# ffs97/deep-mixture-vae

Hardware: AMD Instinct MI355X
Metric: images/sec (train), MNIST K=10 z=64 batch=4096/GPU bf16 (higher is better)
Workload: dtype bf16; 1 GPU; configs[1]: DMVAE MLP 784-500-500-(2000|2000)-z64/K10-2000-500-500-784, one ELBO training step (gather+fwd+loss+bwd+Adam), synthetic rows resident in HBM; per_gpu_batch=4096, global_batch=4096, parallelism=dp1, rccl_ranks=0, multi_rank_rccl_verified_before_this_run=False, hip_graph=True, float_atomics=False, update=adam fused into the dW launch, mode=exact (expectation over q(c|x), priors.py:130-145)

## Files before the change

### deep-mixture-vae_amd/csrc/gemm_bf16.hip

```cpp
#include <algorithm>
#include <cmath>
#include <functional>
#include <map>
#include <mutex>
#include <string>
#include <vector>

#include "gemm_tile.h"
#include "measure.h"

MEAS_TABLES_BF16

namespace dmvae {

template <int BM, int BN, int LAYOUT, int EPI, int NSTAGE, int NW, int BKT = BK, bool CONV = false, bool BONLY = false>
__device__ __forceinline__ void gemm_bf16_body(const GemmArgs& a, const int bid_raw, const int gstart, const int nwg, bf16_t* smem,
                                               const dmvae_adam_ctx* ac = nullptr, const int kslice = -1) {
    constexpr bool A_KC = (LAYOUT != DMVAE_GEMM_DW);
    constexpr bool B_KC = (LAYOUT == DMVAE_GEMM_DX);
    constexpr int A_ELEMS = BM * BKT, B_ELEMS = BN * BKT, STAGE = A_ELEMS + B_ELEMS;
    constexpr int WM = NW / 2;
    constexpr int TM = BM / (16 * WM), TN = BN / 32;
    static_assert(!BONLY || (LAYOUT == DMVAE_GEMM_DW && EPI == DMVAE_EPI_STORE_F32 && !CONV), "bias-only strips: dense DW / STORE_F32");
    constexpr int LOADS = ((BONLY ? 0 : BM) + BN) * BKT / (512 * NW);
    static_assert(NSTAGE >= 2 && NSTAGE <= 8 && LOADS * (NSTAGE - 1) <= 63, "ring depth / vmcnt range");

    MEAS_ANAT(0);
    const int tid = threadIdx.x, lane = tid & 63;
    const int wave = __builtin_amdgcn_readfirstlane(tid >> 6);
    const int wm = wave >> 1, wn = wave & 1;
    const int tiles_n = a.N / BN;
    const int bid = nwg < 0 ? bid_raw : xcd_run_index(gstart + bid_raw, gstart, gstart + nwg);
    int tm, tn;
    {
        const int tiles_m = a.M / BM, gm_max = a.group_m;
        const int gsz = gm_max * tiles_n, grp = bid / gsz, first = grp * gm_max;
        const int gm = min(tiles_m - first, gm_max), in = bid - grp * gsz;
        tm = first + in % gm;
        tn = in / gm;
    }
    const int m0 = tm * BM, n0 = tn * BN;
    const int kbeg = (kslice >= 0 ? kslice : (int)blockIdx.y) * a.k_split;
    const int nk = a.k_split / BKT;

    const bf16_t* Ag = reinterpret_cast<const bf16_t*>(a.A);
    const bf16_t* Bg = reinterpret_cast<const bf16_t*>(a.B);
    if (!A_KC && CONV)
        Ag += ((int64_t)kbeg - (a.conv_p + 1)) * a.lda;
    else
        Ag += A_KC ? ((int64_t)m0 * a.lda + kbeg) : ((int64_t)kbeg * a.lda + m0);
    Bg += B_KC ? ((int64_t)n0 * a.ldb + kbeg) : ((int64_t)kbeg * a.ldb + n0);
    const int64_t stepA = A_KC ? (int64_t)BKT : (int64_t)BKT * a.lda;
    const int64_t stepB = B_KC ? (int64_t)BKT : (int64_t)BKT * a.ldb;

    f32x4 acc[TM][TN];
#pragma unroll
    for (int i = 0; i < TM; ++i)
#pragma unroll
        for (int j = 0; j < TN; ++j) acc[i][j] = f32x4{0.f, 0.f, 0.f, 0.f};
    constexpr bool DW = (LAYOUT == DMVAE_GEMM_DW);
    const bool do_bias = DW && !MEAS_NO_BIAS_MFMA && a.epi.out2 != nullptr && (tm == 0 || BONLY);
    f32x4 bacc[TN];
#pragma unroll
    for (int j = 0; j < TN; ++j) bacc[j] = f32x4{0.f, 0.f, 0.f, 0.f};
    const s16x8 ones_bits = {0x3F80, 0x3F80, 0x3F80, 0x3F80, 0x3F80, 0x3F80, 0x3F80, 0x3F80};
    const bf16x8 ones = __builtin_bit_cast(bf16x8, ones_bits);

    unsigned goA[BM * BKT / (512 * NW)], goB[BN * BKT / (512 * NW)];
    stage_offsets<BM, A_KC, NW, BKT>(a.lda, wave, lane, goA);
    stage_offsets<BN, B_KC, NW, BKT>(a.ldb, wave, lane, goB);
    unsigned selA[BM * BKT / (512 * NW)];
#pragma unroll
    for (int i = 0; i < BM * BKT / (512 * NW); ++i) selA[i] = 0;
    if constexpr (CONV) {
        static_assert(A_KC || BM == 64, "conv-mode weight gradient: 64-row tiles");
#pragma unroll
        for (int i = 0; i < BM * BKT / (512 * NW); ++i) {
            const int row = i * (8 * NW) + wave * 8 + (lane >> 3);
            if constexpr (A_KC) {
                const int k = swz_kc(row, lane & 7) * 8;
                selA[i] = (unsigned)(k / a.conv_c);
                goA[i] = 2u * (unsigned)(row * (int)a.lda + k % a.conv_c);
            } else {
                const int m = m0 + swz_nc<64>(row, lane & 7) * 8;
                const int tap = min(m / a.conv_c, 8);
                goA[i] = 2u * (unsigned)((row + (tap / 3 - 1) * a.conv_p + (tap % 3 - 1) + a.conv_p + 1) * (int)a.lda + m % a.conv_c);
            }
        }
    }
    unsigned short foA[BKT / 32][TM][2], foB[BKT / 32][TN][2];
#pragma unroll
    for (int ks = 0; ks < BKT / 32; ++ks) {
#pragma unroll
        for (int i = 0; i < TM; ++i) frag_offsets<BM, A_KC>(wm * (BM / WM) + i * 16, ks, lane, foA[ks][i][0], foA[ks][i][1]);
#pragma unroll
        for (int j = 0; j < TN; ++j) frag_offsets<BN, B_KC>(wn * (BN / 2) + j * 16, ks, lane, foB[ks][j][0], foB[ks][j][1]);
    }
    const unsigned lds_w = __builtin_amdgcn_readfirstlane(
        (unsigned)(size_t)((__attribute__((address_space(3))) bf16_t*)smem) + 1024u * (unsigned)wave);

    int cv_tap = 0, cv_c0 = 0;
    int64_t cv_off = 0;
    unsigned cv_delta = 0;
    auto issue = [&](int t, int slot) {
        const int tc = t;
        const unsigned s = lds_w + 2u * (unsigned)(slot * STAGE);
        if constexpr (A_KC && CONV) {
            if (t < nk) {
                const int t0 = min(cv_tap, 8), t1 = min(cv_tap + 1, 8);
                cv_off = conv_tap_offset(t0, cv_c0, a.conv_p, a.lda);
                cv_delta = (unsigned)(2 * (int)(conv_tap_offset(t1, 0, a.conv_p, a.lda) - conv_tap_offset(t0, 0, a.conv_p, a.lda)));
                cv_c0 += BKT;
                while (cv_c0 >= a.conv_c) { cv_c0 -= a.conv_c; ++cv_tap; }
            }
            unsigned o[BM * BKT / (512 * NW)];
#pragma unroll
            for (int i = 0; i < BM * BKT / (512 * NW); ++i) o[i] = goA[i] + selA[i] * cv_delta;
            glds_tile(Ag + cv_off, o, s, 1024u * NW);
        } else if constexpr (!BONLY) {
            glds_tile(Ag + tc * stepA, goA, s, 1024u * NW);
        }
        glds_tile(Bg + tc * stepB, goB, s + 2u * A_ELEMS, 1024u * NW);
    };
    auto rd = [&](int slot, int ks, bf16x8 (&af)[TM], bf16x8 (&bfr)[TN]) {
        const bf16_t* As = smem + slot * STAGE;
        const bf16_t* Bs = As + A_ELEMS;
        if constexpr (MEAS_NO_LDS_READ) {
#pragma unroll
            for (int i = 0; i < TM; ++i) af[i] = ones;
#pragma unroll
            for (int j = 0; j < TN; ++j) bfr[j] = ones;
        } else {
            if constexpr (!BONLY) {
#pragma unroll
                for (int i = 0; i < TM; ++i) af[i] = read_frag<A_KC>(As, foA[ks][i][0], foA[ks][i][1]);
            }
#pragma unroll
            for (int j = 0; j < TN; ++j) bfr[j] = read_frag<B_KC>(Bs, foB[ks][j][0], foB[ks][j][1]);
        }
    };
    auto mma = [&](const bf16x8 (&af)[TM], const bf16x8 (&bfr)[TN]) {
        if constexpr (MEAS_NO_MFMA) {
#pragma unroll
            for (int i = 0; i < TM; ++i) asm volatile("" ::"v"(af[i]));
#pragma unroll
            for (int j = 0; j < TN; ++j) asm volatile("" ::"v"(bfr[j]));
        } else if constexpr (!BONLY) {
            __builtin_amdgcn_s_setprio(1);
#pragma unroll
            for (int i = 0; i < TM; ++i)
#pragma unroll
                for (int j = 0; j < TN; ++j)
                    acc[i][j] = __builtin_amdgcn_mfma_f32_16x16x32_bf16(bfr[j], af[i], acc[i][j], 0, 0, 0);
            __builtin_amdgcn_s_setprio(0);
        }
        if constexpr (DW) {
            if (do_bias) {
#pragma unroll
                for (int j = 0; j < TN; ++j) bacc[j] = __builtin_amdgcn_mfma_f32_16x16x32_bf16(bfr[j], ones, bacc[j], 0, 0, 0);
            }
        }
    };

    static_assert(BKT == 64, "the pipelined loop handles two 32-deep sub-steps per ring slot");
    bf16x8 f0a[TM], f0b[TN], f1a[TM], f1b[TN];
    constexpr int NQ = BM * (BN / 4) / (64 * NW);
    float4 target[EPI == DMVAE_EPI_BIAS_RECON ? NQ : 1];
    unsigned target_zero = 0;
    if constexpr (EPI == DMVAE_EPI_BIAS_RECON) {
        const bool tg = (a.epi.recon_kind & 0x100) != 0;
        int64_t tfirst = 0;
        if (tg) {
            const dmvae_state* tst = reinterpret_cast<const dmvae_state*>(a.epi.aux2);
            tfirst = tst ? (int64_t)tst->batch_cursor * a.epi.d_off : a.epi.ld1;
        }
        if (tg) {
            const int32_t* perm = reinterpret_cast<const int32_t*>(a.epi.aux1);
            int64_t src[NQ];
            bool ok[NQ];
#pragma unroll
            for (int q = 0; q < NQ; ++q) {
                const int idx = q * (64 * NW) + tid;
                const int m = m0 + idx / (BN / 4), n = n0 + (idx % (BN / 4)) * 4;
                const int64_t sr = tfirst + m;
                ok[q] = m < a.epi.m_valid && n + 3 < (int)a.epi.ld0 && sr >= 0 && sr < a.epi.ld2;
                src[q] = ok[q] ? sr : 0;
            }
            if (perm) {
#pragma unroll
                for (int q = 0; q < NQ; ++q) src[q] = (int64_t)perm[src[q]];
            }
#pragma unroll
            for (int q = 0; q < NQ; ++q) {
                const int idx = q * (64 * NW) + tid;
                const int n = n0 + (idx % (BN / 4)) * 4;
                ok[q] = ok[q] && src[q] >= 0 && src[q] < a.epi.ld2;
                target[q] = *reinterpret_cast<const float4*>(reinterpret_cast<const float*>(a.epi.aux0) + (ok[q] ? src[q] * a.epi.ld0 + n : 0));
                if (!ok[q]) target_zero |= 1u << q;
            }
        } else {
#pragma unroll
            for (int q = 0; q < NQ; ++q) {
                const int idx = q * (64 * NW) + tid;
                const int ml = idx / (BN / 4), c = idx % (BN / 4);
                target[q] = *reinterpret_cast<const float4*>(reinterpret_cast<const float*>(a.epi.aux0) + (int64_t)(m0 + ml) * a.epi.ld0 + n0 + c * 4);
            }
        }
    }
    constexpr bool LAT_PRE = EPI == DMVAE_EPI_LATENT && NQ <= 4;
    float lat[LAT_PRE ? NQ : 1][12];
    if constexpr (LAT_PRE) {
#pragma unroll
        for (int q = 0; q < NQ; ++q) {
            const int idx = q * (64 * NW) + tid;
            const int ml = idx / (BN / 4), c = idx % (BN / 4);
            loadf4(a.epi.aux0, (int64_t)(m0 + ml) * a.epi.ld0 + n0 + c * 4, lat[q]);
            loadf4(a.epi.aux1, (int64_t)(m0 + ml) * a.epi.ld1 + n0 + c * 4, lat[q] + 4);
            loadf4(a.epi.aux2, (int64_t)(m0 + ml) * a.epi.ld2 + n0 + c * 4, lat[q] + 8);
        }
    }
    constexpr bool HAS_BIAS = (EPI == DMVAE_EPI_BIAS_RELU || EPI == DMVAE_EPI_BIAS_F32 || EPI == DMVAE_EPI_BIAS_SIGMOID || EPI == DMVAE_EPI_BIAS_RECON);
    static_assert((64 * NW) % (BN / 4) == 0, "a thread keeps its column block across the epilogue's passes");
    float bq[4] = {0.f, 0.f, 0.f, 0.f};
    if constexpr (HAS_BIAS) loadf4(a.epi.bias, n0 + (tid % (BN / 4)) * 4, bq);
    uint2 gate[EPI == DMVAE_EPI_RELU_MASK ? NQ : 1];
    if constexpr (EPI == DMVAE_EPI_RELU_MASK) {
#pragma unroll
        for (int q = 0; q < NQ; ++q) {
            const int idx = q * (64 * NW) + tid;
            const int ml = idx / (BN / 4), c = idx % (BN / 4);
            if constexpr (MEAS_NO_MASK_READ) gate[q] = make_uint2(0x3f803f80u, 0x3f803f80u);
            else gate[q] = *reinterpret_cast<const uint2*>(reinterpret_cast<const bf16_t*>(a.epi.aux0) + (int64_t)(m0 + ml) * a.epi.ld0 + n0 + c * 4);
        }
    }
#pragma unroll
    for (int t = 0; t < NSTAGE; ++t)
        if (t < nk) issue(t, t);
    if (nk >= NSTAGE) wait_vmcnt<LOADS*(NSTAGE - 1)>();
    else wait_vmcnt<0>();
    __builtin_amdgcn_s_barrier();
    MEAS_ANAT(1);
    rd(0, 0, f0a, f0b);
    for (int kt = 0; kt < nk; kt += NSTAGE) {
#pragma unroll
        for (int s = 0; s < NSTAGE; ++s) {
            if (kt + s < nk) {
                rd(s, 1, f1a, f1b);
                mma(f0a, f0b);
                asm volatile("s_waitcnt lgkmcnt(0)" ::: "memory");
                if (kt + s + NSTAGE <= nk) wait_vmcnt<LOADS*(NSTAGE - 2)>();
                else wait_vmcnt<0>();
                __builtin_amdgcn_s_barrier();
                if constexpr (!MEAS_NO_KLOOP_LOADS) {
                    if (kt + s + NSTAGE < nk) issue(kt + s + NSTAGE, s);
                }
                if (kt + s + 1 < nk) rd((s + 1) % NSTAGE, 0, f0a, f0b);
                mma(f1a, f1b);
            }
        }
    }
    wait_vmcnt<0>();
    __builtin_amdgcn_s_barrier();
    MEAS_KLOOP_END();
    MEAS_ANAT(2);

    float loss = 0.f;
    const int li = lane & 15, g = lane >> 4;
    constexpr int CH = BN / 4, NT = 64 * NW;
    static_assert(BM * BN * 4 <= NSTAGE * STAGE * 2, "fp32 tile must fit in the ring");
    dmvae_epilogue epi_s = a.epi;
    if constexpr (EPI == DMVAE_EPI_STORE_F32 && (CONV || LAYOUT == DMVAE_GEMM_DW)) {
        const int ys = kslice >= 0 ? kslice : (int)blockIdx.y;
        epi_s.out = reinterpret_cast<float*>(epi_s.out) + (int64_t)ys * a.slab_stride;
        if (epi_s.out2) epi_s.out2 = reinterpret_cast<float*>(epi_s.out2) + (int64_t)ys * a.slab_stride2;
    }
    float* ct = reinterpret_cast<float*>(smem);
    if constexpr (MEAS_NO_EPILOGUE) {
#pragma unroll
        for (int i = 0; i < TM; ++i)
#pragma unroll
            for (int j = 0; j < TN; ++j) asm volatile("" ::"v"(acc[i][j]));
    } else if constexpr (!BONLY) {
#pragma unroll
    for (int i = 0; i < TM; ++i)
#pragma unroll
        for (int j = 0; j < TN; ++j) {
            const int ml = wm * (BM / WM) + i * 16 + li;
            const int c = (wn * (BN / 2) + j * 16) / 4 + g;
            *reinterpret_cast<f32x4*>(ct + ml * BN + ((c ^ (ml & 7)) << 2)) = acc[i][j];
        }
    __syncthreads();
    constexpr int KSPLIT_MAX_S = 8;
    constexpr bool KSLICE_OK = !CONV && LAYOUT != DMVAE_GEMM_DW && BM * BN <= 4096 && NW <= 4 && BM * BN * 4 + 16 <= NSTAGE * STAGE * 2 &&
                               (EPI == DMVAE_EPI_BIAS_RELU || EPI == DMVAE_EPI_RELU_MASK || EPI == DMVAE_EPI_BIAS_F32 || EPI == DMVAE_EPI_LATENT);
    if constexpr (KSLICE_OK) {
        if (a.tick != nullptr && gridDim.y > 1) {
            const int S = (int)gridDim.y, tile_lin = tm * tiles_n + tn;
            constexpr int Q = BM * BN;
            static_assert(KSPLIT_MAX_S == 8, "the combine issues eight loads per quad");
            f32x4* slab0 = reinterpret_cast<f32x4*>(a.ws) + (int64_t)tile_lin * S * (Q / 4);
            const f32x4* ct4 = reinterpret_cast<const f32x4*>(ct);
            for (int q = tid; q < Q / 4; q += 64 * NW) {
                const f32x4 v = ct4[q];
                f32x4* dst = slab0 + (int64_t)blockIdx.y * (Q / 4) + q;
                asm volatile("global_store_dwordx4 %0, %1, off sc1" ::"v"(dst), "v"(v) : "memory");
            }
            asm volatile("s_waitcnt vmcnt(0)" ::: "memory");
            __syncthreads();
            int* flag = reinterpret_cast<int*>(ct + BM * BN);
            if (tid == 0) *flag = __hip_atomic_fetch_add(a.tick + tile_lin, 1, __ATOMIC_RELAXED, __HIP_MEMORY_SCOPE_AGENT);
            __syncthreads();
            if (*flag != S - 1) return;
            for (int q = tid; q < Q / 4; q += 64 * NW) {
                const f32x4 *p0, *p1, *p2, *p3, *p4, *p5, *p6, *p7;
                auto at = [&](int sl) { return slab0 + (int64_t)(sl < S ? sl : S - 1) * (Q / 4) + q; };
                p0 = at(0); p1 = at(1); p2 = at(2); p3 = at(3); p4 = at(4); p5 = at(5); p6 = at(6); p7 = at(7);
                f32x4 u0, u1, u2, u3, u4, u5, u6, u7;
                asm volatile(
                    "global_load_dwordx4 %0, %8, off sc1\n\tglobal_load_dwordx4 %1, %9, off sc1\n\tglobal_load_dwordx4 %2, %10, off sc1\n\tglobal_load_dwordx4 %3, %11, off sc1\n\t"
                    "global_load_dwordx4 %4, %12, off sc1\n\tglobal_load_dwordx4 %5, %13, off sc1\n\tglobal_load_dwordx4 %6, %14, off sc1\n\tglobal_load_dwordx4 %7, %15, off sc1\n\t"
                    "s_waitcnt vmcnt(0)"
                    : "=&v"(u0), "=&v"(u1), "=&v"(u2), "=&v"(u3), "=&v"(u4), "=&v"(u5), "=&v"(u6), "=&v"(u7)
                    : "v"(p0), "v"(p1), "v"(p2), "v"(p3), "v"(p4), "v"(p5), "v"(p6), "v"(p7)
                    : "memory");
                f32x4 v = u0;
                if (1 < S) v += u1;
                if (2 < S) v += u2;
                if (3 < S) v += u3;
                if (4 < S) v += u4;
                if (5 < S) v += u5;
                if (6 < S) v += u6;
                if (7 < S) v += u7;
                reinterpret_cast<f32x4*>(ct)[q] = v;
            }
            if (tid == 0) __hip_atomic_store(a.tick + tile_lin, 0, __ATOMIC_RELAXED, __HIP_MEMORY_SCOPE_AGENT);
            __syncthreads();
        }
    }
    if constexpr (EPI == DMVAE_EPI_ADAM && !CONV) {
        constexpr int NQE = BM * CH / NT;
        constexpr int NB = NQE % 4 == 0 ? 4 : (NQE % 2 == 0 ? 2 : 1);
        const unsigned base = (unsigned)((reinterpret_cast<const float*>(a.epi.out) - ac->grad) + (int64_t)m0 * a.epi.ldo + n0);
#ifndef DMVAE_ADAM_EPI_BATCHWISE
#ifdef DMVAE_ADAM_EPI_NB
        constexpr int PNB = NQE % DMVAE_ADAM_EPI_NB == 0 ? DMVAE_ADAM_EPI_NB : NB, PDEPTH = DMVAE_ADAM_EPI_DEPTH;
#else
        constexpr int PNB = NB, PDEPTH = 2;
#endif
        adam_pipelined<PNB, NQE / PNB, PDEPTH>(*ac,
            [&](int i, int b) {
                const int idx = (i * PNB + b) * NT + tid;
                return base + (unsigned)(idx / CH) * (unsigned)a.epi.ldo + (unsigned)(idx % CH) * 4u;
            },
            [&](int i, int b, float (&gv)[4]) {
                const int idx = (i * PNB + b) * NT + tid;
                const int ml = idx / CH, c = idx % CH;
                const f32x4 t = *reinterpret_cast<const f32x4*>(ct + ml * BN + ((c ^ (ml & 7)) << 2));
                gv[0] = t[0]; gv[1] = t[1]; gv[2] = t[2]; gv[3] = t[3];
            });
#else
#pragma unroll
        for (int q0 = 0; q0 < NQE; q0 += NB) {
            unsigned off[NB];
#pragma unroll
            for (int b = 0; b < NB; ++b) {
                const int idx = (q0 + b) * NT + tid;
                off[b] = base + (unsigned)(idx / CH) * (unsigned)a.epi.ldo + (unsigned)(idx % CH) * 4u;
            }
            adam_quads<NB>(*ac, off, [&](int b, float (&gv)[4]) {
                const int idx = (q0 + b) * NT + tid;
                const int ml = idx / CH, c = idx % CH;
                const f32x4 t = *reinterpret_cast<const f32x4*>(ct + ml * BN + ((c ^ (ml & 7)) << 2));
                gv[0] = t[0]; gv[1] = t[1]; gv[2] = t[2]; gv[3] = t[3];
            });
        }
#endif
    } else
#pragma unroll
    for (int q = 0; q < BM * CH / NT; ++q) {
        const int idx = q * NT + tid;
        const int ml = idx / CH, c = idx % CH;
        bool padcol = false;
        if constexpr (CONV) {
            padcol = n0 + c * 4 >= a.epi.n_valid;
            if (padcol && !(EPI == DMVAE_EPI_STORE_F32 && a.slab_stride)) continue;
        }
        const f32x4 t = *reinterpret_cast<const f32x4*>(ct + ml * BN + ((c ^ (ml & 7)) << 2));
        float v[4] = {t[0], t[1], t[2], t[3]};
        if (padcol) { v[0] = 0.f; v[1] = 0.f; v[2] = 0.f; v[3] = 0.f; }
        if constexpr (EPI == DMVAE_EPI_ADAM) {
            const int64_t off = (reinterpret_cast<const float*>(a.epi.out) - ac->grad) + (int64_t)(m0 + ml) * a.epi.ldo + n0 + c * 4;
            adam_quad(*ac, off, v);
        } else if constexpr (EPI == DMVAE_EPI_RELU_MASK) {
            const uint2 y = gate[q];
            v[0] = __uint_as_float(y.x << 16) > 0.f ? v[0] : 0.f;
            v[1] = __uint_as_float(y.x & 0xffff0000u) > 0.f ? v[1] : 0.f;
            v[2] = __uint_as_float(y.y << 16) > 0.f ? v[2] : 0.f;
            v[3] = __uint_as_float(y.y & 0xffff0000u) > 0.f ? v[3] : 0.f;
            ActIO<bf16_t>::store4(a.epi.out, (int64_t)(m0 + ml) * a.epi.ldo + n0 + c * 4, v);
        } else if constexpr (EPI == DMVAE_EPI_BIAS_RECON) {
            const bool tz = (target_zero >> q) & 1u;
            const float xq[4] = {tz ? 0.f : target[q].x, tz ? 0.f : target[q].y, tz ? 0.f : target[q].z, tz ? 0.f : target[q].w};
            epilogue_quad<EPI, bf16_t>(a.epi, m0 + ml, n0 + c * 4, v, loss, xq, nullptr, bq);
        } else if constexpr (LAT_PRE) {
            epilogue_quad<EPI, bf16_t>(a.epi, m0 + ml, n0 + c * 4, v, loss, lat[q]);
        } else {
            epilogue_quad<EPI, bf16_t>(epi_s, m0 + ml, n0 + c * 4, v, loss, nullptr, nullptr, HAS_BIAS ? bq : nullptr);
        }
    }
    }
    if constexpr (DW) {
        if (do_bias && wm == 0 && li == 0) {
            float* db = reinterpret_cast<float*>(epi_s.out2);
#pragma unroll
            for (int j = 0; j < TN; ++j) {
                const int n = n0 + wn * (BN / 2) + j * 16 + g * 4;
                if constexpr (CONV) {
                    if (n >= a.epi.n_valid) {
                        if (EPI == DMVAE_EPI_STORE_F32 && a.slab_stride2) *reinterpret_cast<float4*>(db + n) = make_float4(0.f, 0.f, 0.f, 0.f);
                        continue;
                    }
                }
                if constexpr (EPI == DMVAE_EPI_ATOMIC_F32) {
#pragma unroll
                    for (int e = 0; e < 4; ++e) atomicAdd(db + n + e, bacc[j][e]);
                } else if constexpr (EPI == DMVAE_EPI_ADAM) {
                    float v[4] = {bacc[j][0], bacc[j][1], bacc[j][2], bacc[j][3]};
                    adam_quad(*ac, (db - ac->grad) + n, v);
                } else {
                    *reinterpret_cast<float4*>(db + n) = make_float4(bacc[j][0], bacc[j][1], bacc[j][2], bacc[j][3]);
                }
            }
        }
    }
    if constexpr (EPI == DMVAE_EPI_BIAS_RECON) {
        float* red = reinterpret_cast<float*>(smem);
        lds_barrier();
        const float t = block_sum_waves<NW>(loss, red);
        constexpr int CM = BM / 64, CN = BN / 64;
        if (tid < CM * CN) a.epi.partials[(tm * CM + tid / CN) * (a.N / 64) + tn * CN + tid % CN] = tid == 0 ? t : 0.f;
    }
    MEAS_ANAT_DRAIN();
}

template <int BM, int BN, int LAYOUT, int EPI, int NSTAGE, int NW>
__global__ __launch_bounds__(64 * NW, (EPI == DMVAE_EPI_BIAS_RECON ? 1 : NW / 2)) void gemm_bf16_kernel(GemmArgs a) {
    __shared__ __attribute__((aligned(16))) bf16_t smem[NSTAGE * (BM + BN) * BK];
    gemm_bf16_body<BM, BN, LAYOUT, EPI, NSTAGE, NW>(a, blockIdx.x, 0, gridDim.x, smem);
}

template <int BM, int BN, int EPI, int NSTAGE, int NW>
__global__ __launch_bounds__(64 * NW, NW / 2) void gemm_bf16_dx_riders_kernel(GemmArgs a, GemmRiders r) {
    __shared__ __attribute__((aligned(16))) bf16_t smem[NSTAGE * (BM + BN) * BK];
    const int lead = r.nfin + (r.gat_last ? 0 : r.ngat);
    if (blockIdx.y > 0 && ((int)blockIdx.x < lead || (r.gat_last && (int)blockIdx.x >= (int)gridDim.x - r.ngat))) return;
    if (r.gat_last && (int)blockIdx.x >= (int)gridDim.x - r.ngat) {
        if constexpr (MEAS_EMPTY_GATHER_RIDERS) return;
        gather_rows_block<bf16_t, 16>((int)blockIdx.x - ((int)gridDim.x - r.ngat), 64 * NW, r.gat);
        return;
    }
    if ((int)blockIdx.x < r.nfin) {
        if (NW > 4 && threadIdx.x >= 256) return;
        if ((int)blockIdx.x < r.fin.nblocks) step_finalize_block((int)blockIdx.x, r.fin, reinterpret_cast<float(*)[17]>(smem));
        return;
    }
    if ((int)blockIdx.x < lead) {
        if constexpr (MEAS_EMPTY_GATHER_RIDERS) return;
        gather_rows_block<bf16_t, 16>((int)blockIdx.x - r.nfin, 64 * NW, r.gat);
        return;
    }
    gemm_bf16_body<BM, BN, DMVAE_GEMM_DX, EPI, NSTAGE, NW>(a, (int)blockIdx.x - lead, lead, (int)gridDim.x - lead - (r.gat_last ? r.ngat : 0), smem);
}

template <int BM, int BN, int LAYOUT, int EPI, int NSTAGE, int NW>
__global__ __launch_bounds__(64 * NW, NW / 2) void gemm_bf16_conv_kernel(GemmArgs a) {
    __shared__ __attribute__((aligned(16))) bf16_t smem[NSTAGE * (BM + BN) * BK];
    if constexpr (LAYOUT == DMVAE_GEMM_DW) {
        if ((gridDim.y & 7) == 0) {
            const int L = (int)(blockIdx.y * gridDim.x + blockIdx.x), xcd = L & 7, j = L >> 3, T = (int)gridDim.x;
            gemm_bf16_body<BM, BN, LAYOUT, EPI, NSTAGE, NW, BK, true>(a, j % T, 0, -1, smem, nullptr, (j / T) * 8 + xcd);
            return;
        }
    }
    gemm_bf16_body<BM, BN, LAYOUT, EPI, NSTAGE, NW, BK, true>(a, blockIdx.x, 0, gridDim.x, smem);
}

void* gemm_bf16_anatomy() { return MEAS_SYMBOL(g_anat); }
void* gemm_bf16_stamps() { return MEAS_SYMBOL(g_stamps); }
struct GroupedArgs {
    int nprob;
    int kind[DMVAE_MAX_GROUP];
    int start[DMVAE_MAX_GROUP + 1];
    int cls_start[DMVAE_MAX_GROUP], cls_end[DMVAE_MAX_GROUP];
    int nsl[DMVAE_MAX_GROUP];
    GemmArgs p[DMVAE_MAX_GROUP];
    dmvae_adam_ctx adam;
    dmvae_finalize_args fin;
    int lead, lead_work;
    int xcut, xr0[8], xcnt[8];
};
template <int BM, int BN, int LAYOUT, int EPI, int NSTAGE, int NW = 4, bool SHORTK = false>
__global__ __launch_bounds__(64 * NW, NW == 8 ? 4 : 1) void gemm_bf16_grouped_kernel(GroupedArgs g) {
    __shared__ __attribute__((aligned(16))) bf16_t smem[SHORTK ? 2 * (64 + 64) * BK : 3 * (128 + 64) * BK];
    const dmvae_adam_ctx* ac = EPI == DMVAE_EPI_ADAM ? &g.adam : nullptr;
    if constexpr (EPI == DMVAE_EPI_ADAM) {
        if ((int)blockIdx.x < g.lead) {
            if ((int)blockIdx.x >= g.lead_work) return;
            const int64_t n4 = g.adam.seg_n >> 2;
            for (int64_t q = (int64_t)blockIdx.x * (64 * NW) + threadIdx.x; q < n4; q += (int64_t)g.lead_work * (64 * NW)) {
                const int64_t off = g.adam.seg_off + 4 * q;
                const float4 gq = *reinterpret_cast<const float4*>(g.adam.grad + off);
                const float gv[4] = {gq.x, gq.y, gq.z, gq.w};
                adam_quad(g.adam, off, gv);
            }
            return;
        }
    }
    int bx = (int)blockIdx.x;
    if constexpr (EPI == DMVAE_EPI_ADAM) bx -= g.lead;
    if constexpr (EPI == DMVAE_EPI_RELU_MASK) {
        if (bx < g.lead) {
            if (NW > 4 && threadIdx.x >= 256) return;
            if (bx < g.fin.nblocks) step_finalize_block(bx, g.fin, reinterpret_cast<float(*)[17]>(smem));
            return;
        }
        bx -= g.lead;
    }
    int i = 0, item;
    if (g.xcut) {
        const int x = bx & 7, j = bx >> 3;
        if (j >= g.xcnt[x]) return;
        item = g.xr0[x] + j;
    } else {
        while (i + 1 < g.nprob && bx >= g.start[i + 1]) ++i;
        item = g.cls_start[i] + xcd_run_index(bx, g.cls_start[i], g.cls_end[i]);
    }
    i = 0;
    while (i + 1 < g.nprob && item >= g.start[i + 1]) ++i;
    int bid = item - g.start[i];
    const int kind = g.kind[i];
    const int gs = 0, cnt = -1;
    int ksl = -1;
    if (g.nsl[i] > 1) {
        const int tiles_i = (g.start[i + 1] - g.start[i]) / g.nsl[i];
        ksl = bid / tiles_i;
        bid -= ksl * tiles_i;
    }
    MEAS_WG_BEGIN();
    if constexpr (SHORTK) {
        gemm_bf16_body<64, 64, LAYOUT, EPI, 2, NW>(g.p[i], bid, gs, cnt, smem, ac, ksl);
    } else {
        if (kind == 0) gemm_bf16_body<128, 128, LAYOUT, EPI, 2, NW>(g.p[i], bid, gs, cnt, smem, ac, ksl);
        else if (kind == 1) gemm_bf16_body<128, 64, LAYOUT, EPI, 3, NW>(g.p[i], bid, gs, cnt, smem, ac, ksl);
        else if (kind == 3) {
            if constexpr (LAYOUT == DMVAE_GEMM_DW && EPI == DMVAE_EPI_STORE_F32)
                gemm_bf16_body<64, 64, LAYOUT, EPI, 4, NW, BK, false, true>(g.p[i], bid, gs, cnt, smem, ac, ksl);
        }
        else gemm_bf16_body<BM, BN, LAYOUT, EPI, NSTAGE, NW>(g.p[i], bid, gs, cnt, smem, ac, ksl);
    }
    MEAS_WG_END(LAYOUT, kind);
}

static int g_thin = 2;
static int g_group_m = 0;
int gemm_auto_group_m(int tiles_m, int tiles_n, int bm, int bn, double run) {
    if (g_group_m > 0) return g_group_m;
    const double R = run > 0.0 ? run : std::max(1.0, tiles_m * (double)tiles_n / 8.0);
    int gm = (int)(std::sqrt(R * bn / bm) + 0.5);
    const int need = (int)((R + tiles_n - 1) / tiles_n);
    gm = std::max(gm, need);
    return std::max(1, std::min(gm, tiles_m));
}
static int g_shortk = 0;
static int g_conv_short = 2;
static int g_grouped_cls = 1;
static int g_dx_group_nw = 0;
static int g_grouped_mixed = 1;
static int g_grouped_xcut = 0;
template <int BM, int BN, int LAYOUT, int EPI, int NSTAGE, int NW = 4>
static const char* kernel_name(bool grouped) {
    static char nm[2][64];
    static bool init = false;
    if (!init) {
        snprintf(nm[0], 64, "gemm_bf16_kernel<%d, %d, %d, %d, %d, %d>", BM, BN, LAYOUT, EPI, NSTAGE, NW);
        snprintf(nm[1], 64, "gemm_bf16_grouped_kernel<%d, %d, %d, %d, %d, %d>", BM, BN, LAYOUT, EPI, NSTAGE, NW);
        init = true;
    }
    return nm[grouped ? 1 : 0];
}
static double gemm_bytes(const GemmArgs& a, int layout = DMVAE_GEMM_FWD) {
    const int k = a.epi.kind;
    if (k == DMVAE_EPI_ADAM) return 2.0 * ((double)a.M * a.K + (double)a.K * a.N);
    const double osz = (k == DMVAE_EPI_STORE_F32 || k == DMVAE_EPI_ATOMIC_F32 || k == DMVAE_EPI_BIAS_F32 || k == DMVAE_EPI_BIAS_SIGMOID) ? 4.0 : 2.0;
    if (a.conv_c) {
// ... 400 lines not shown
```

### deep-mixture-vae_amd/csrc/gemm_epilogue.h

```cpp
#pragma once
#include "common.h"

namespace dmvae {

struct GemmArgs {
    const void* A; int64_t lda;
    const void* B; int64_t ldb;
    int M, N, K, k_split;
    int group_m;
    int conv_p, conv_c;
    dmvae_epilogue epi;
    float* ws = nullptr; int64_t ws_elems = 0;
    int64_t slab_stride = 0;
    int64_t slab_stride2 = 0;
    float* csum_out = nullptr; int64_t csum_ld = 0;
    const float* csum_in = nullptr; int csum_rows = 0;
    int bias_only = 0;
    int* tick = nullptr;
};

__host__ __device__ __forceinline__ int64_t conv_tap_offset(int tap, int c0, int P, int64_t lda) {
    return (int64_t)((tap / 3 - 1) * P + (tap % 3 - 1)) * lda + c0;
}

template <typename T> struct ActIO;
template <> struct ActIO<bf16_t> {
    static __device__ __forceinline__ void store4(void* base, int64_t off, const float v[4]) {
        uint2 p;
        p.x = pack2bf(v[0], v[1]);
        p.y = pack2bf(v[2], v[3]);
        *reinterpret_cast<uint2*>(reinterpret_cast<bf16_t*>(base) + off) = p;
    }
    static __device__ __forceinline__ void load4(const void* base, int64_t off, float v[4]) {
        const uint2 p = *reinterpret_cast<const uint2*>(reinterpret_cast<const bf16_t*>(base) + off);
        v[0] = __uint_as_float(p.x << 16);
        v[1] = __uint_as_float(p.x & 0xffff0000u);
        v[2] = __uint_as_float(p.y << 16);
        v[3] = __uint_as_float(p.y & 0xffff0000u);
    }
};
template <> struct ActIO<float> {
    static __device__ __forceinline__ void store4(void* base, int64_t off, const float v[4]) {
        *reinterpret_cast<float4*>(reinterpret_cast<float*>(base) + off) = make_float4(v[0], v[1], v[2], v[3]);
    }
    static __device__ __forceinline__ void load4(const void* base, int64_t off, float v[4]) {
        const float4 p = *reinterpret_cast<const float4*>(reinterpret_cast<const float*>(base) + off);
        v[0] = p.x; v[1] = p.y; v[2] = p.z; v[3] = p.w;
    }
};

__device__ __forceinline__ void loadf4(const void* base, int64_t off, float v[4]) {
    ActIO<float>::load4(base, off, v);
}

__device__ __forceinline__ float xent_logits(float l, float x) {
    return fmaxf(l, 0.f) - l * x + log1pf(__expf(-fabsf(l)));
}
__device__ __forceinline__ float sigmoidf_(float l) { return 1.0f / (1.0f + __expf(-l)); }
struct dmvae_gather_args {
    const float* data; int64_t n_rows; int dim; const int32_t* perm;
    int64_t first; int batch, n_valid, B_pad;
    void* out_act; int64_t ld_act; float* out_f32; int64_t ld_f32; int cols_pad;
    const dmvae_state* st;
    int nblocks;
};
template <typename ACT, int U, bool PERM>
__device__ __forceinline__ void gather_rows_pass(const int base, const int nthreads, const int total, const int quads, const int64_t first, const dmvae_gather_args& g) {
    int r[U], c[U];
    int64_t idx[U];
    bool inb[U];
#pragma unroll
    for (int u = 0; u < U; ++u) {
        const int i = base + u * nthreads;
        r[u] = i < total ? i / quads : -1;
        c[u] = i < total ? (i - r[u] * quads) * 4 : 0;
        const int64_t sr = first + r[u];
        inb[u] = r[u] >= 0 && r[u] < g.n_valid && sr >= 0 && sr < g.n_rows;
        idx[u] = inb[u] ? sr : 0;
    }
    if constexpr (PERM) {
#pragma unroll
        for (int u = 0; u < U; ++u) idx[u] = (int64_t)g.perm[idx[u]];
    }
    float4 q[U];
#pragma unroll
    for (int u = 0; u < U; ++u) {
        inb[u] = inb[u] && idx[u] >= 0 && idx[u] < g.n_rows && c[u] < g.dim;
        q[u] = *reinterpret_cast<const float4*>(g.data + (inb[u] ? idx[u] * g.dim + c[u] : 0));
    }
#pragma unroll
    for (int u = 0; u < U; ++u) {
        if (r[u] < 0) continue;
        const float v[4] = {inb[u] ? q[u].x : 0.f, inb[u] ? q[u].y : 0.f, inb[u] ? q[u].z : 0.f, inb[u] ? q[u].w : 0.f};
        if (g.out_act) ActIO<ACT>::store4(g.out_act, (int64_t)r[u] * g.ld_act + c[u], v);
        if (g.out_f32) ActIO<float>::store4(g.out_f32, (int64_t)r[u] * g.ld_f32 + c[u], v);
    }
}
template <typename ACT, int U = 8>
__device__ __forceinline__ void gather_rows_block(const int bx, const int nthreads, const dmvae_gather_args& g) {
    int64_t first = g.first;
    if (g.st) first = (int64_t)g.st->batch_cursor * g.batch;
    const int quads = g.cols_pad >> 2;
    const int total = g.B_pad * quads;
    if (g.dim % 4 == 0 && (reinterpret_cast<uintptr_t>(g.data) & 15) == 0 && g.n_rows > 0) {
        for (int base = bx * nthreads * U + (int)threadIdx.x; base < total; base += g.nblocks * nthreads * U) {
            if (g.perm) gather_rows_pass<ACT, U, true>(base, nthreads, total, quads, first, g);
            else gather_rows_pass<ACT, U, false>(base, nthreads, total, quads, first, g);
        }
        return;
    }
    for (int i = bx * nthreads + (int)threadIdx.x; i < total; i += g.nblocks * nthreads) {
        const int r = i / quads, c = (i - r * quads) * 4;
        float v[4] = {0.f, 0.f, 0.f, 0.f};
        if (r < g.n_valid) {
            int64_t src = first + r;
            if (g.perm) src = (src >= 0 && src < g.n_rows) ? (int64_t)g.perm[src] : -1;
            if (src >= 0 && src < g.n_rows) {
                const float* p = g.data + src * g.dim + c;
#pragma unroll
                for (int j = 0; j < 4; ++j) v[j] = (c + j < g.dim) ? p[j] : 0.f;
            }
        }
        if (g.out_act) ActIO<ACT>::store4(g.out_act, (int64_t)r * g.ld_act + c, v);
        if (g.out_f32) ActIO<float>::store4(g.out_f32, (int64_t)r * g.ld_f32 + c, v);
    }
}

struct GemmRiders {
    dmvae_finalize_args fin; int nfin = 0;
    dmvae_gather_args gat; int ngat = 0;
    int gat_last = 0;
};

__device__ __forceinline__ void xent_sigmoid(float l, float x, float& xent, float& sig) {
    const float e = __expf(-fabsf(l));
    const float inv = __frcp_rn(1.0f + e);
    xent = fmaxf(l, 0.f) - l * x + __logf(1.0f + e);
    sig = l >= 0.f ? inv : e * inv;
}

template <int EPI, typename ACT>
__device__ __forceinline__ void epilogue_quad(const dmvae_epilogue& e, int m, int n, float v[4], float& loss, const float* xpre = nullptr, float* stored = nullptr,
                                              const float* bpre = nullptr, const float* ypre = nullptr) {
    if constexpr (EPI == DMVAE_EPI_BIAS_RELU) {
        float b[4];
        if (bpre) { b[0] = bpre[0]; b[1] = bpre[1]; b[2] = bpre[2]; b[3] = bpre[3]; }
        else loadf4(e.bias, n, b);
#pragma unroll
        for (int j = 0; j < 4; ++j) v[j] = fmaxf(v[j] + b[j], 0.f);
        ActIO<ACT>::store4(e.out, (int64_t)m * e.ldo + n, v);
    } else if constexpr (EPI == DMVAE_EPI_BIAS_F32) {
        float b[4];
        if (bpre) { b[0] = bpre[0]; b[1] = bpre[1]; b[2] = bpre[2]; b[3] = bpre[3]; }
        else loadf4(e.bias, n, b);
#pragma unroll
        for (int j = 0; j < 4; ++j) v[j] += b[j];
        ActIO<float>::store4(e.out, (int64_t)m * e.ldo + n, v);
    } else if constexpr (EPI == DMVAE_EPI_BIAS_SIGMOID) {
        float b[4];
        if (bpre) { b[0] = bpre[0]; b[1] = bpre[1]; b[2] = bpre[2]; b[3] = bpre[3]; }
        else loadf4(e.bias, n, b);
#pragma unroll
        for (int j = 0; j < 4; ++j) v[j] = sigmoidf_(v[j] + b[j]);
        ActIO<float>::store4(e.out, (int64_t)m * e.ldo + n, v);
    } else if constexpr (EPI == DMVAE_EPI_BIAS_RECON) {
        float b[4], x[4], d[4];
        if (bpre) { b[0] = bpre[0]; b[1] = bpre[1]; b[2] = bpre[2]; b[3] = bpre[3]; }
        else loadf4(e.bias, n, b);
        if (xpre) { x[0] = xpre[0]; x[1] = xpre[1]; x[2] = xpre[2]; x[3] = xpre[3]; }
        else loadf4(e.aux0, (int64_t)m * e.ld0 + n, x);
        const bool rowok = m < e.m_valid;
#pragma unroll
        for (int j = 0; j < 4; ++j) {
            const float l = v[j] + b[j];
            v[j] = l;
            const bool ok = rowok && (n + j) < e.n_valid;
            if ((e.recon_kind & 0xff) == 0) {
                float xe, sg;
                xent_sigmoid(l, x[j], xe, sg);
                loss += ok ? xe : 0.f;
                d[j] = ok ? (sg - x[j]) * e.scale : 0.f;
            } else {
                const float r = l - x[j];
                loss += ok ? 0.5f * r * r : 0.f;
                d[j] = ok ? r * e.scale : 0.f;
            }
        }
        ActIO<ACT>::store4(e.out, (int64_t)m * e.ldo + n, d);
        if (stored) { stored[0] = d[0]; stored[1] = d[1]; stored[2] = d[2]; stored[3] = d[3]; }
        if (e.out2) ActIO<float>::store4(e.out2, (int64_t)m * e.ldo2 + n, v);
    } else if constexpr (EPI == DMVAE_EPI_RELU_MASK) {
        float y[4];
        if (ypre) { y[0] = ypre[0]; y[1] = ypre[1]; y[2] = ypre[2]; y[3] = ypre[3]; }
        else ActIO<ACT>::load4(e.aux0, (int64_t)m * e.ld0 + n, y);
#pragma unroll
        for (int j = 0; j < 4; ++j) v[j] = y[j] > 0.f ? v[j] : 0.f;
        ActIO<ACT>::store4(e.out, (int64_t)m * e.ldo + n, v);
        if (stored) { stored[0] = v[0]; stored[1] = v[1]; stored[2] = v[2]; stored[3] = v[3]; }
    } else if constexpr (EPI == DMVAE_EPI_LATENT) {
        float gm[4], gl[4], cl[4], o0[4], o1[4];
        if (xpre) {
#pragma unroll
            for (int j = 0; j < 4; ++j) { gm[j] = xpre[j]; gl[j] = xpre[4 + j]; cl[j] = xpre[8 + j]; }
        } else {
            loadf4(e.aux0, (int64_t)m * e.ld0 + n, gm);
            loadf4(e.aux1, (int64_t)m * e.ld1 + n, gl);
            loadf4(e.aux2, (int64_t)m * e.ld2 + n, cl);
        }
#pragma unroll
        for (int j = 0; j < 4; ++j) {
            o0[j] = v[j] + gm[j];
            o1[j] = v[j] * cl[j] + gl[j];
        }
        ActIO<ACT>::store4(e.out, (int64_t)m * e.ldo + n, o0);
        ActIO<ACT>::store4(e.out, (int64_t)m * e.ldo + e.d_off + n, o1);
    } else if constexpr (EPI == DMVAE_EPI_STORE_F32) {
        ActIO<float>::store4(e.out, (int64_t)m * e.ldo + n, v);
    } else if constexpr (EPI == DMVAE_EPI_ATOMIC_F32) {
        float* o = reinterpret_cast<float*>(e.out) + (int64_t)m * e.ldo + n;
#pragma unroll
        for (int j = 0; j < 4; ++j) atomicAdd(o + j, v[j]);
    }
}

}
```

### deep-mixture-vae_amd/csrc/measure.h

```cpp
#pragma once

#ifndef DMVAE_ABLATE
#define DMVAE_ABLATE 0
#endif

namespace dmvae {
constexpr bool MEAS_NO_MFMA = DMVAE_ABLATE == 1 || DMVAE_ABLATE == 4;
constexpr bool MEAS_NO_LDS_READ = DMVAE_ABLATE == 2 || DMVAE_ABLATE == 4;
constexpr bool MEAS_NO_KLOOP_LOADS = DMVAE_ABLATE == 3;
constexpr bool MEAS_NO_EPILOGUE = DMVAE_ABLATE == 5;
constexpr bool MEAS_NO_MASK_READ = DMVAE_ABLATE == 8;
constexpr bool MEAS_NO_BIAS_MFMA = DMVAE_ABLATE == 9;
constexpr bool MEAS_STAMPS = DMVAE_ABLATE == 6;
constexpr bool MEAS_NO_STEP_GATHER = DMVAE_ABLATE == 11;
constexpr bool MEAS_EMPTY_GATHER_RIDERS = DMVAE_ABLATE == 12;
}

#if DMVAE_ABLATE == 6
#define MEAS_TABLES_BF16                                  \
    __device__ unsigned long long g_mid[2048];            \
    __device__ unsigned long long g_anat[2048 * 8];       \
    __device__ unsigned long long g_stamps[2048 * 4];
#define MEAS_HWID() (((unsigned long long)__builtin_amdgcn_s_getreg((31 << 11) | 4) << 32) | (unsigned)__builtin_amdgcn_s_getreg((3 << 11) | 20))
#define MEAS_ANAT(i) do { if (threadIdx.x == 0 && blockIdx.x < 2048) g_anat[blockIdx.x * 8 + (i)] = __builtin_amdgcn_s_memrealtime(); } while (0)
#define MEAS_KLOOP_END() do { if (threadIdx.x == 0 && blockIdx.x < 2048) g_mid[blockIdx.x] = __builtin_amdgcn_s_memrealtime(); } while (0)
#define MEAS_ANAT_DRAIN()                                                                             \
    do {                                                                                              \
        MEAS_ANAT(3);                                                                                 \
        asm volatile("s_waitcnt vmcnt(0)" ::: "memory");                                              \
        MEAS_ANAT(4);                                                                                 \
        if (threadIdx.x == 0 && blockIdx.x < 2048) g_anat[blockIdx.x * 8 + 5] = MEAS_HWID();          \
    } while (0)
#define MEAS_WG_BEGIN() const unsigned long long meas_t0_ = __builtin_amdgcn_s_memrealtime()
#define MEAS_WG_END(layout, kind)                                                                                          \
    do {                                                                                                                   \
        if (threadIdx.x == 0 && blockIdx.x < 2048) {                                                                       \
            unsigned long long* st_ = g_stamps + 4 * blockIdx.x;                                                           \
            st_[0] = meas_t0_;                                                                                             \
            st_[1] = __builtin_amdgcn_s_memrealtime();                                                                     \
            st_[2] = MEAS_HWID();                                                                                          \
            st_[3] = ((g_mid[blockIdx.x] - meas_t0_) << 16) | ((unsigned long long)(layout) << 8) | (unsigned)(kind);       \
        }                                                                                                                  \
    } while (0)
#define MEAS_TABLES_256 __device__ unsigned long long g_anat256[4096 * 8];
#define MEAS_ANAT256(i)                                                                                  \
    do {                                                                                                 \
        if (threadIdx.x == 0 && blockIdx.x < 4096) {                                                     \
            g_anat256[blockIdx.x * 8 + (i)] = __builtin_amdgcn_s_memrealtime();                          \
            if ((i) < 2) g_anat256[blockIdx.x * 8 + 4 + (i)] = __builtin_amdgcn_s_memtime();             \
        }                                                                                                \
    } while (0)
#define MEAS_ANAT256_DRAIN()                                                                             \
    do {                                                                                                 \
        asm volatile("s_waitcnt vmcnt(0)" ::: "memory");                                                 \
        __syncthreads();                                                                                 \
        MEAS_ANAT256(2);                                                                                 \
        if (threadIdx.x == 0 && blockIdx.x < 4096) g_anat256[blockIdx.x * 8 + 3] = MEAS_HWID();          \
    } while (0)
#define MEAS_SYMBOL(sym) ([] { void* p_ = nullptr; return hipGetSymbolAddress(&p_, HIP_SYMBOL(sym)) == hipSuccess ? p_ : nullptr; }())
#else
#define MEAS_TABLES_BF16
#define MEAS_TABLES_256
#define MEAS_ANAT(i) do { } while (0)
#define MEAS_KLOOP_END() do { } while (0)
#define MEAS_ANAT_DRAIN() do { } while (0)
#define MEAS_WG_BEGIN() do { } while (0)
#define MEAS_WG_END(layout, kind) do { } while (0)
#define MEAS_ANAT256(i) do { } while (0)
#define MEAS_ANAT256_DRAIN() do { } while (0)
#define MEAS_SYMBOL(sym) (static_cast<void*>(nullptr))
#endif

#if DMVAE_ABLATE == 10
#define MEAS_TABLES_HDX __device__ unsigned long long g_hdx[1024 * 16];
#define MEAS_HDX_BEGIN() unsigned long long hx_[12] = {}; unsigned long long hx_last_; hx_[0] = __builtin_amdgcn_s_memtime(); hx_[10] = __builtin_amdgcn_s_memrealtime()
#define MEAS_HDX_MARK(i) do { hx_last_ = __builtin_amdgcn_s_memtime(); hx_[i] = hx_last_; } while (0)
#define MEAS_HDX_ACC(i) do { const unsigned long long t_ = __builtin_amdgcn_s_memtime(); hx_[i] += t_ - hx_last_; hx_last_ = t_; } while (0)
#define MEAS_HDX_END(steps)                                                                                                        \
    do {                                                                                                                           \
        MEAS_HDX_MARK(3);                                                                                                          \
        asm volatile("s_waitcnt vmcnt(0)" ::: "memory");                                                                           \
        MEAS_HDX_MARK(4);                                                                                                          \
        hx_[11] = __builtin_amdgcn_s_memrealtime();                                                                                \
        if (threadIdx.x == 0 && blockIdx.x < 1024) {                                                                               \
            for (int i_ = 0; i_ < 12; ++i_) g_hdx[blockIdx.x * 16 + i_] = hx_[i_];                                                 \
            g_hdx[blockIdx.x * 16 + 13] = (unsigned long long)(steps);                                                             \
            g_hdx[blockIdx.x * 16 + 12] = (((unsigned long long)__builtin_amdgcn_s_getreg((31 << 11) | 4) << 32) | (unsigned)__builtin_amdgcn_s_getreg((3 << 11) | 20)); \
        }                                                                                                                          \
    } while (0)
#define MEAS_SYMBOL_HDX(sym) ([] { void* p_ = nullptr; return hipGetSymbolAddress(&p_, HIP_SYMBOL(sym)) == hipSuccess ? p_ : nullptr; }())
#else
#define MEAS_TABLES_HDX
#define MEAS_HDX_BEGIN() do { } while (0)
#define MEAS_HDX_MARK(i) do { } while (0)
#define MEAS_HDX_ACC(i) do { } while (0)
#define MEAS_HDX_END(steps) do { } while (0)
#define MEAS_SYMBOL_HDX(sym) (static_cast<void*>(nullptr))
#endif

#if DMVAE_ABLATE == 7
#define MEAS_LAT_STAMP(i) do { if (blockIdx.x == 0 && threadIdx.x == 0) reinterpret_cast<unsigned long long*>(L.a.loss_partials + 2 * gridDim.x)[i] = __builtin_amdgcn_s_memrealtime(); } while (0)
#else
#define MEAS_LAT_STAMP(i) do { } while (0)
#endif
```

Measured before the change: 15.03 million images/sec.

## Overlap reconstruction-target gather with the K-loop in the recon GEMM epilogue

The recon-loss GEMM used to load its gathered fp32 target rows, including the permutation lookups, before the K-loop and wait on them up front. Now the permutation indices are read per wave through constant-address-space loads and shared across lanes by row. The target float4 loads are issued late in the K-loop, with vmcnt waits adjusted so they complete under the last MFMA steps. This hides the target-fetch latency behind compute, at the cost of more registers held across the loop and more involved vmcnt accounting. New ablation switches for the target fetch and recon store are also added for measurement.

```diff
diff --git a/deep-mixture-vae_amd/csrc/gemm_bf16.hip b/deep-mixture-vae_amd/csrc/gemm_bf16.hip
--- a/deep-mixture-vae_amd/csrc/gemm_bf16.hip
+++ b/deep-mixture-vae_amd/csrc/gemm_bf16.hip
@@ -4,6 +4,7 @@
 #include <map>
 #include <mutex>
 #include <string>
+#include <type_traits>
 #include <vector>
 
 #include "gemm_tile.h"
@@ -23,7 +24,7 @@
     constexpr int TM = BM / (16 * WM), TN = BN / 32;
     static_assert(!BONLY || (LAYOUT == DMVAE_GEMM_DW && EPI == DMVAE_EPI_STORE_F32 && !CONV), "bias-only strips: dense DW / STORE_F32");
     constexpr int LOADS = ((BONLY ? 0 : BM) + BN) * BKT / (512 * NW);
-    static_assert(NSTAGE >= 2 && NSTAGE <= 8 && LOADS * (NSTAGE - 1) <= 63, "ring depth / vmcnt range");
+    static_assert(NSTAGE >= 2 && NSTAGE <= 8 && LOADS * (NSTAGE - 1) + (EPI == DMVAE_EPI_BIAS_RECON ? BM * (BN / 4) / (64 * NW) : 0) <= 63, "ring depth / vmcnt range");
 
     MEAS_ANAT(0);
     const int tid = threadIdx.x, lane = tid & 63;
@@ -165,48 +166,91 @@
     static_assert(BKT == 64, "the pipelined loop handles two 32-deep sub-steps per ring slot");
     bf16x8 f0a[TM], f0b[TN], f1a[TM], f1b[TN];
     constexpr int NQ = BM * (BN / 4) / (64 * NW);
-    float4 target[EPI == DMVAE_EPI_BIAS_RECON ? NQ : 1];
+    constexpr bool TGT = EPI == DMVAE_EPI_BIAS_RECON;
+    constexpr int TGT_X = TGT && !MEAS_NO_TARGET_FETCH ? NQ : 0;
+    constexpr int TROWS = 64 / (BN / 4);
+    static_assert(!TGT || 64 % (BN / 4) == 0, "a wave's quads of one pass lie in whole rows");
+    float4 target[TGT ? NQ : 1];
     unsigned target_zero = 0;
-    if constexpr (EPI == DMVAE_EPI_BIAS_RECON) {
-        const bool tg = (a.epi.recon_kind & 0x100) != 0;
-        int64_t tfirst = 0;
+    int tsrc[TGT ? NQ : 1];
+    const bool tg = TGT && (a.epi.recon_kind & 0x100) != 0;
+    int64_t tfirst = 0;
+    if constexpr (TGT) {
         if (tg) {
             const dmvae_state* tst = reinterpret_cast<const dmvae_state*>(a.epi.aux2);
             tfirst = tst ? (int64_t)tst->batch_cursor * a.epi.d_off : a.epi.ld1;
         }
-        if (tg) {
-            const int32_t* perm = reinterpret_cast<const int32_t*>(a.epi.aux1);
-            int64_t src[NQ];
-            bool ok[NQ];
+    }
+    if constexpr (TGT) {
+#pragma unroll
+        for (int q = 0; q < NQ; ++q) { target[q] = make_float4(0.f, 0.f, 0.f, 0.f); tsrc[q] = -1; }
+    }
+    auto target_rows = [&](auto has_perm) {
+        if constexpr (TGT && !MEAS_NO_TARGET_FETCH) {
+            typedef const __attribute__((address_space(4))) int32_t* cperm_t;
+            const cperm_t perm = (cperm_t)reinterpret_cast<uintptr_t>(a.epi.aux1);
+            const int myr = lane / (BN / 4);
+            const int64_t tb = tfirst + m0;
+            if (decltype(has_perm)::value && tb >= 0 && tb + BM <= a.epi.ld2 && a.epi.ld2 <= 0x7fffffff) {
+                const cperm_t pw = perm + tb + wave * TROWS;
+                int pe[NQ][TROWS];
+#pragma unroll
+                for (int q = 0; q < NQ; ++q)
+#pragma unroll
+                    for (int r = 0; r < TROWS; ++r) pe[q][r] = pw[q * (64 * NW / (BN / 4)) + r];
+#pragma unroll
+                for (int q = 0; q < NQ; ++q) {
+                    int src = -1;
+#pragma unroll
+                    for (int r = 0; r < TROWS; ++r) {
+                        const int m = m0 + q * (64 * NW / (BN / 4)) + wave * TROWS + r;
+                        const int row = m < a.epi.m_valid && (unsigned)pe[q][r] < (unsigned)a.epi.ld2 ? pe[q][r] : -1;
+                        src = myr == r ? row : src;
+                    }
+                    tsrc[q] = src;
+                }
+                return;
+            }
+#pragma unroll
+            for (int q = 0; q < NQ; ++q) {
+                int src = -1;
+#pragma unroll
+                for (int r = 0; r < TROWS; ++r) {
+                    const int m = m0 + q * (64 * NW / (BN / 4)) + wave * TROWS + r;
+                    const int64_t sr = tfirst + m;
+                    const bool okr = m < a.epi.m_valid && sr >= 0 && sr < a.epi.ld2;
+                    int64_t pe = okr ? sr : 0;
+                    if constexpr (decltype(has_perm)::value) pe = (int64_t)perm[pe];
+                    const int row = okr && pe >= 0 && pe < a.epi.ld2 && pe <= 0x7fffffff ? (int)pe : -1;
+                    src = myr == r ? row : src;
+                }
+                tsrc[q] = src;
+            }
+        }
+    };
+    const float* tptr[TGT ? NQ : 1];
+    auto target_addrs = [&]() {
+        if constexpr (TGT && !MEAS_NO_TARGET_FETCH) {
 #pragma unroll
             for (int q = 0; q < NQ; ++q) {
                 const int idx = q * (64 * NW) + tid;
-                const int m = m0 + idx / (BN / 4), n = n0 + (idx % (BN / 4)) * 4;
-                const int64_t sr = tfirst + m;
-                ok[q] = m < a.epi.m_valid && n + 3 < (int)a.epi.ld0 && sr >= 0 && sr < a.epi.ld2;
-                src[q] = ok[q] ? sr : 0;
-            }
-            if (perm) {
-#pragma unroll
-                for (int q = 0; q < NQ; ++q) src[q] = (int64_t)perm[src[q]];
-            }
-#pragma unroll
-            for (int q = 0; q < NQ; ++q) {
-                const int idx = q * (64 * NW) + tid;
-                const int n = n0 + (idx % (BN / 4)) * 4;
-                ok[q] = ok[q] && src[q] >= 0 && src[q] < a.epi.ld2;
-                target[q] = *reinterpret_cast<const float4*>(reinterpret_cast<const float*>(a.epi.aux0) + (ok[q] ? src[q] * a.epi.ld0 + n : 0));
-                if (!ok[q]) target_zero |= 1u << q;
-            }
-        } else {
-#pragma unroll
-            for (int q = 0; q < NQ; ++q) {
-                const int idx = q * (64 * NW) + tid;
-                const int ml = idx / (BN / 4), c = idx % (BN / 4);
-                target[q] = *reinterpret_cast<const float4*>(reinterpret_cast<const float*>(a.epi.aux0) + (int64_t)(m0 + ml) * a.epi.ld0 + n0 + c * 4);
-            }
-        }
-    }
+                const int ml = idx / (BN / 4), n = n0 + (idx % (BN / 4)) * 4;
+                if (tg) {
+                    const bool ok = tsrc[q] >= 0 && n + 3 < (int)a.epi.ld0;
+                    tptr[q] = reinterpret_cast<const float*>(a.epi.aux0) + (ok ? (int64_t)tsrc[q] * a.epi.ld0 + n : 0);
+                    if (!ok) target_zero |= 1u << q;
+                } else {
+                    tptr[q] = reinterpret_cast<const float*>(a.epi.aux0) + (int64_t)(m0 + ml) * a.epi.ld0 + n;
+                }
+            }
+        }
+    };
+    auto issue_targets = [&]() {
+        if constexpr (TGT && !MEAS_NO_TARGET_FETCH) {
+#pragma unroll
+            for (int q = 0; q < NQ; ++q) target[q] = *reinterpret_cast<const float4*>(tptr[q]);
+        }
+    };
     constexpr bool LAT_PRE = EPI == DMVAE_EPI_LATENT && NQ <= 4;
     float lat[LAT_PRE ? NQ : 1][12];
     if constexpr (LAT_PRE) {
@@ -236,8 +280,17 @@
 #pragma unroll
     for (int t = 0; t < NSTAGE; ++t)
         if (t < nk) issue(t, t);
-    if (nk >= NSTAGE) wait_vmcnt<LOADS*(NSTAGE - 1)>();
-    else wait_vmcnt<0>();
+    if constexpr (TGT_X != 0) {
+        if (tg) { if (a.epi.aux1) target_rows(std::true_type()); else target_rows(std::false_type()); }
+        target_addrs();
+        if (nk <= NSTAGE) issue_targets();
+        if (nk > NSTAGE) wait_vmcnt<LOADS*(NSTAGE - 1)>();
+        else if (nk == NSTAGE) wait_vmcnt<LOADS*(NSTAGE - 1) + TGT_X>();
+        else wait_vmcnt<TGT_X>();
+    } else {
+        if (nk >= NSTAGE) wait_vmcnt<LOADS*(NSTAGE - 1)>();
+        else wait_vmcnt<0>();
+    }
     __builtin_amdgcn_s_barrier();
     MEAS_ANAT(1);
     rd(0, 0, f0a, f0b);
@@ -248,18 +301,27 @@
                 rd(s, 1, f1a, f1b);
                 mma(f0a, f0b);
                 asm volatile("s_waitcnt lgkmcnt(0)" ::: "memory");
-                if (kt + s + NSTAGE <= nk) wait_vmcnt<LOADS*(NSTAGE - 2)>();
-                else wait_vmcnt<0>();
+                if constexpr (TGT_X != 0) {
+                    if (kt + s + NSTAGE < nk) wait_vmcnt<LOADS*(NSTAGE - 2)>();
+                    else if (kt + s + NSTAGE == nk) wait_vmcnt<LOADS*(NSTAGE - 2) + TGT_X>();
+                    else wait_vmcnt<TGT_X>();
+                } else {
+                    if (kt + s + NSTAGE <= nk) wait_vmcnt<LOADS*(NSTAGE - 2)>();
+                    else wait_vmcnt<0>();
+                }
                 __builtin_amdgcn_s_barrier();
                 if constexpr (!MEAS_NO_KLOOP_LOADS) {
                     if (kt + s + NSTAGE < nk) issue(kt + s + NSTAGE, s);
                 }
+                if constexpr (TGT_X != 0) {
+                    if (kt + s + NSTAGE == nk - 1) issue_targets();
+                }
                 if (kt + s + 1 < nk) rd((s + 1) % NSTAGE, 0, f0a, f0b);
                 mma(f1a, f1b);
             }
         }
     }
-    wait_vmcnt<0>();
+    wait_vmcnt<TGT_X>();
     __builtin_amdgcn_s_barrier();
     MEAS_KLOOP_END();
     MEAS_ANAT(2);
@@ -290,6 +352,7 @@
             *reinterpret_cast<f32x4*>(ct + ml * BN + ((c ^ (ml & 7)) << 2)) = acc[i][j];
         }
     __syncthreads();
+    MEAS_ANAT(6);
     constexpr int KSPLIT_MAX_S = 8;
     constexpr bool KSLICE_OK = !CONV && LAYOUT != DMVAE_GEMM_DW && BM * BN <= 4096 && NW <= 4 && BM * BN * 4 + 16 <= NSTAGE * STAGE * 2 &&
                                (EPI == DMVAE_EPI_BIAS_RELU || EPI == DMVAE_EPI_RELU_MASK || EPI == DMVAE_EPI_BIAS_F32 || EPI == DMVAE_EPI_LATENT);
diff --git a/deep-mixture-vae_amd/csrc/gemm_epilogue.h b/deep-mixture-vae_amd/csrc/gemm_epilogue.h
--- a/deep-mixture-vae_amd/csrc/gemm_epilogue.h
+++ b/deep-mixture-vae_amd/csrc/gemm_epilogue.h
@@ -1,5 +1,6 @@
 #pragma once
 #include "common.h"
+#include "measure.h"
 
 namespace dmvae {
 
@@ -186,7 +187,7 @@
                 d[j] = ok ? r * e.scale : 0.f;
             }
         }
-        ActIO<ACT>::store4(e.out, (int64_t)m * e.ldo + n, d);
+        if constexpr (!MEAS_NO_RECON_STORE) ActIO<ACT>::store4(e.out, (int64_t)m * e.ldo + n, d);
         if (stored) { stored[0] = d[0]; stored[1] = d[1]; stored[2] = d[2]; stored[3] = d[3]; }
         if (e.out2) ActIO<float>::store4(e.out2, (int64_t)m * e.ldo2 + n, v);
     } else if constexpr (EPI == DMVAE_EPI_RELU_MASK) {
diff --git a/deep-mixture-vae_amd/csrc/measure.h b/deep-mixture-vae_amd/csrc/measure.h
--- a/deep-mixture-vae_amd/csrc/measure.h
+++ b/deep-mixture-vae_amd/csrc/measure.h
@@ -14,22 +14,29 @@
 constexpr bool MEAS_STAMPS = DMVAE_ABLATE == 6;
 constexpr bool MEAS_NO_STEP_GATHER = DMVAE_ABLATE == 11;
 constexpr bool MEAS_EMPTY_GATHER_RIDERS = DMVAE_ABLATE == 12;
+constexpr bool MEAS_NO_TARGET_FETCH = DMVAE_ABLATE == 14;
+constexpr bool MEAS_NO_RECON_STORE = DMVAE_ABLATE == 15;
 }
 
-#if DMVAE_ABLATE == 6
+#if DMVAE_ABLATE == 6 || DMVAE_ABLATE == 13
 #define MEAS_TABLES_BF16                                  \
     __device__ unsigned long long g_mid[2048];            \
     __device__ unsigned long long g_anat[2048 * 8];       \
     __device__ unsigned long long g_stamps[2048 * 4];
 #define MEAS_HWID() (((unsigned long long)__builtin_amdgcn_s_getreg((31 << 11) | 4) << 32) | (unsigned)__builtin_amdgcn_s_getreg((3 << 11) | 20))
-#define MEAS_ANAT(i) do { if (threadIdx.x == 0 && blockIdx.x < 2048) g_anat[blockIdx.x * 8 + (i)] = __builtin_amdgcn_s_memrealtime(); } while (0)
-#define MEAS_KLOOP_END() do { if (threadIdx.x == 0 && blockIdx.x < 2048) g_mid[blockIdx.x] = __builtin_amdgcn_s_memrealtime(); } while (0)
+#if DMVAE_ABLATE == 13
+#define MEAS_ANAT_HERE (EPI == DMVAE_EPI_BIAS_RECON)
+#else
+#define MEAS_ANAT_HERE true
+#endif
+#define MEAS_ANAT(i) do { if (MEAS_ANAT_HERE && threadIdx.x == 0 && blockIdx.x < 2048) g_anat[blockIdx.x * 8 + (i)] = __builtin_amdgcn_s_memrealtime(); } while (0)
+#define MEAS_KLOOP_END() do { if (MEAS_ANAT_HERE && threadIdx.x == 0 && blockIdx.x < 2048) g_mid[blockIdx.x] = __builtin_amdgcn_s_memrealtime(); } while (0)
 #define MEAS_ANAT_DRAIN()                                                                             \
     do {                                                                                              \
         MEAS_ANAT(3);                                                                                 \
         asm volatile("s_waitcnt vmcnt(0)" ::: "memory");                                              \
         MEAS_ANAT(4);                                                                                 \
-        if (threadIdx.x == 0 && blockIdx.x < 2048) g_anat[blockIdx.x * 8 + 5] = MEAS_HWID();          \
+        if (MEAS_ANAT_HERE && threadIdx.x == 0 && blockIdx.x < 2048) g_anat[blockIdx.x * 8 + 5] = MEAS_HWID(); \
     } while (0)
 #define MEAS_WG_BEGIN() const unsigned long long meas_t0_ = __builtin_amdgcn_s_memrealtime()
 #define MEAS_WG_END(layout, kind)                                                                                          \
```

Result: no change. 14.97 million images/sec (-0.4%).
